# aliabdelkader/FusionTransformer

Hardware: AMD Instinct MI355X
Metric: frames/sec fwd+bwd (SemanticKITTI synth), whole job (higher is better)
Workload: dtype f32

## Files before the change

fusiontransformer_amd/_lib.py:

```python
from __future__ import annotations

import ctypes as C
import os

import torch

_HERE = os.path.dirname(os.path.abspath(__file__))
LIB_PATH = os.path.join(_HERE, "csrc", "libftx.so")

_i32, _i64, _f32, _vp, _sz = C.c_int32, C.c_int64, C.c_float, C.c_void_p, C.c_size_t

SIGNATURES = {
    "ftx_version": (C.c_int, []),
    "ftx_last_error": (C.c_char_p, []),
    "ftx_stream_scratch_bytes": (_sz, []),
    "ftx_stream_scratch_attach": (C.c_int, [_vp, _vp, _sz]),
    "ftx_stream_scratch_reset": (C.c_int, [_vp]),
    "ftx_stream_scratch_release": (C.c_int, [_vp]),
    "ftx_hash": (C.c_int, [_vp, _i64, _vp, _vp]),
    "ftx_hash_kernel": (C.c_int, [_vp, _i64, _vp, _i32, _vp, _vp]),
    "ftx_floor_coords": (C.c_int, [_vp, _i64, _i32, _vp, _vp]),
    "ftx_hashtable_capacity": (_i64, [_i64]),
    "ftx_hashtable_build": (C.c_int, [_vp, _i64, _vp, _vp, _i64, _vp]),
    "ftx_hashtable_query": (C.c_int, [_vp, _i64, _vp, _vp, _i64, _vp, _vp]),
# ... 75 lines not shown
    "ftx_bn_train_fwd": (C.c_int, [_vp, _vp, _vp, _vp, _vp, _vp, _f32, _f32, _i64, _i32, _i32, _vp, _vp, _vp, _vp, _sz, _vp]),
    "ftx_bn_eval_fwd": (C.c_int, [_vp, _vp, _vp, _vp, _vp, _vp, _f32, _i64, _i32, _i32, _vp, _vp]),
    "ftx_adam_chunk_elements": (_i32, []),
    "ftx_adam_tensor_bytes": (_i32, []),
    "ftx_adam_step": (C.c_int, [_vp, _vp, _vp, _i32, C.c_double, C.c_double, _f32, _f32, _vp]),
    "ftx_add_layernorm_fwd": (C.c_int, [_vp, _vp, _vp, _vp, _vp, _f32, _i64, _i32, _vp, _vp, _vp, _vp, _vp]),
    "ftx_layernorm_bwd_workspace_bytes": (_sz, [_i64, _i32]),
    "ftx_add_layernorm_bwd": (C.c_int, [_vp, _vp, _vp, _vp, _vp, _vp, _i64, _i32, _i32, _vp, _vp, _vp, _sz, _vp]),
    "ftx_colsum_workspace_bytes": (_sz, [_i64, _i32]),
    "ftx_colsum": (C.c_int, [_vp, _i64, _i32, _vp, _vp, _sz, _vp]),
    "ftx_attn_fwd": (C.c_int, [_vp, _i32, _i32, _i32, _i32, _f32, _vp, _vp, _vp]),
    "ftx_attn_bwd_workspace_bytes": (_sz, [_i32, _i32, _i32]),
    "ftx_attn_bwd": (C.c_int, [_vp, _vp, _vp, _vp, _i32, _i32, _i32, _i32, _f32, _vp, _vp, _sz, _vp]),
    "ftx_attn_fwd_tiled": (C.c_int, [_vp, _i32, _i32, _i32, _i32, _f32, _vp, _vp, _i32, _i32, _vp]),
    "ftx_attn_bwd_tiled": (C.c_int, [_vp, _vp, _vp, _vp, _i32, _i32, _i32, _i32, _f32, _vp, _vp, _sz, _i32, _i32, _vp]),
    "ftx_attn_fwd_bf16": (C.c_int, [_vp, _i32, _i32, _i32, _i32, _f32, _vp, _vp, _i32, _i32, _vp]),
    "ftx_attn_bwd_bf16": (C.c_int, [_vp, _vp, _vp, _vp, _i32, _i32, _i32, _i32, _f32, _vp, _vp, _sz, _i32, _i32, _vp]),
    "ftx_attn_split_tiling_built": (_i32, [_i32, _i32, _i32]),
    "ftx_attn_fwd_split": (C.c_int, [_vp, _i32, _i32, _i32, _i32, _f32, _vp, _vp, _i32, _i32, _vp]),
    "ftx_attn_bwd_split": (C.c_int, [_vp, _vp, _vp, _vp, _i32, _i32, _i32, _i32, _f32, _vp, _vp, _sz, _i32, _i32, _vp]),
    "ftx_dense_gemm_bf16": (C.c_int, [_vp, _vp, _i32, _vp, _vp, _i64, _i32, _i32, _i32, _vp, _vp, _vp]),
    "ftx_dense_wgrad_bf16_workspace_bytes": (_sz, [_i64, _i32, _i32]),
    "ftx_dense_wgrad_bf16": (C.c_int, [_vp, _vp, _i64, _i32, _i32, _vp, _vp, _sz, _vp]),
    "ftx_dense_bf16_tile": (C.c_int, [_i32, _i64, _i32, _i32, _vp, _vp, _vp]),
    "ftx_dense_gemm_split": (C.c_int, [_vp, _vp, _i32, _vp, _vp, _i64, _i32, _i32, _i32, _vp, _vp, _vp]),
    "ftx_dense_wgrad_split_workspace_bytes": (_sz, [_i64, _i32, _i32]),
    "ftx_dense_wgrad_split": (C.c_int, [_vp, _vp, _i64, _i32, _i32, _vp, _vp, _sz, _vp]),
    "ftx_dense_split_tile": (C.c_int, [_i32, _i64, _i32, _i32, _vp, _vp, _vp]),
    "ftx_fusion_loss_workspace_bytes": (_sz, []),
    "ftx_fusion_loss": (C.c_int, [_vp, _vp, _vp, _vp, _vp, _vp, _f32, _i64, _i32, _i32, _vp, _vp, _vp, _vp, _vp, _vp, _vp, _vp, _sz, _vp]),
# ... 99 lines not shown
```

fusiontransformer_amd/csrc/ftx_attn.hip:

```cpp
#include "ftx_common.h"
#include "ftx_mfma.h"
#include "ftx_split.h"

using namespace ftx;

constexpr int HD = 64;
constexpr int TS = 68;
constexpr float LOG2E = 1.4426950408889634f;
constexpr float LN2 = 0.6931471805599453f;

__device__ inline int acc_row(int g, int h) { return (g & 3) + 8 * (g >> 2) + 4 * h; }

__device__ inline float exp2_raw(float x) { return __builtin_amdgcn_exp2f(x); }

__device__ inline const float *qkv_row(const float *qkv, int b, int t, int which, int hd, int T, int nh) {
  return qkv + ((((int64_t)b * T + t) * 3 + which) * nh + hd) * HD;
}

struct AttnF32 {
  using Frag = float[32];
  template <int NT> using Stage = float4[512 / NT];
  using X = f32x16;
  static constexpr int tile_floats(bool row, bool col) { return 32 * TS; }

// ... 339 lines not shown
#pragma unroll
      for (int t = 0; t < NTILES; ++t)
#pragma unroll
        for (int g = 0; g < 16; ++g) cw[(t * 16 + g) * 64] = acc[t][g];
    }
    __syncthreads();
    if ((grp & (2 * s - 1)) == 0 && grp + s < SPLIT) {
#pragma unroll
      for (int t = 0; t < NTILES; ++t)
#pragma unroll
        for (int g = 0; g < 16; ++g) acc[t][g] += cw[(t * 16 + g) * 64];
    }
  }
}

template <class P, int QW, int SPLIT>
__device__ inline void attn_fwd_body(const float *__restrict__ qkv, int T, int nh, float scale, float *__restrict__ out, float *__restrict__ lse) {
  constexpr int NT = 64 * QW, KF = P::tile_floats(true, false), GROUP = KF + P::tile_floats(false, true);
  __shared__ __attribute__((aligned(16))) float smem[smem_floats<QW, SPLIT, 34, GROUP>()];
  const int tid = threadIdx.x % NT, grp = threadIdx.x / NT;
  float *Ks = smem + grp * GROUP, *Vs = Ks + KF;
  const int wave = tid >> 6, lane = tid & 63, l31 = lane & 31, h = lane >> 5;
  const int hd = blockIdx.y, b = blockIdx.z;
  const int q = blockIdx.x * (32 * QW) + wave * 32 + l31;
  const bool qv = q < T;
  const bool wave_live = blockIdx.x * (32 * QW) + wave * 32 < T;
  const float sl2 = scale * LOG2E;

  typename P::Frag qf;
  P::load_frag(qkv_row(qkv, b, qv ? q : 0, 0, hd, T, nh), h, qv, qf);
  P::fold(qf, sl2);

// ... 16 lines not shown
      P::template prefetch<NT>(qkv, b, hd, 1, (kt + SPLIT) * 32, T, nh, tid, rk);
      P::template prefetch<NT>(qkv, b, hd, 2, (kt + SPLIT) * 32, T, nh, tid, rv);
    }
    if (kt < ntiles && wave_live) {
      f32x16 st;
#pragma unroll
      for (int g = 0; g < 16; ++g) st[g] = 0.f;
      P::first(Ks, l31, h, qf, st);
#pragma unroll
      for (int g = 0; g < 16; ++g) st[g] = P::score(st[g], sl2);
      if (kt == ntiles - 1) {
#pragma unroll
        for (int g = 0; g < 16; ++g)
          if (kt * 32 + acc_row(g, h) >= T) st[g] = -INFINITY;
      }
      float mx = fmaxf(fmaxf(fmaxf(st[0], st[1]), fmaxf(st[2], st[3])), fmaxf(fmaxf(st[4], st[5]), fmaxf(st[6], st[7])));
      mx = fmaxf(mx, fmaxf(fmaxf(fmaxf(st[8], st[9]), fmaxf(st[10], st[11])), fmaxf(fmaxf(st[12], st[13]), fmaxf(st[14], st[15]))));
      mx = fmaxf(mx, __shfl_xor(mx, 32, 64));
      const float m_new = fmaxf(m, mx);
      float rs = 0.f;
#pragma unroll
      for (int g = 0; g < 16; ++g) {
        float p = exp2_raw(st[g] - m_new);
        st[g] = p;
        rs += p;
      }
      rs += __shfl_xor(rs, 32, 64);
      if (__any(m_new != m)) {
        const float alpha = exp2_raw(m - m_new);
        l *= alpha;
// ... 219 lines not shown
    group_sync<QW>();
  }
  merge_sum<QW, SPLIT, 2>(smem, grp, wave, lane, acc);
  if (qv && grp == 0) {
    float *qp = gqkv + ((((int64_t)b * T + q) * 3 + 0) * nh + hd) * HD;
#pragma unroll
    for (int g4 = 0; g4 < 4; ++g4) {
      int r = acc_row(4 * g4, h);
      *(float4 *)(qp + r) = make_float4(acc[0][4 * g4], acc[0][4 * g4 + 1], acc[0][4 * g4 + 2], acc[0][4 * g4 + 3]);
      *(float4 *)(qp + 32 + r) = make_float4(acc[1][4 * g4], acc[1][4 * g4 + 1], acc[1][4 * g4 + 2], acc[1][4 * g4 + 3]);
    }
  }
}

template <int QW, int SPLIT>
__global__ __launch_bounds__(64 * QW * SPLIT) void attn_fwd_kernel(const float *__restrict__ qkv, int T, int nh, float scale, float *__restrict__ out,
    float *__restrict__ lse) {
  attn_fwd_body<AttnF32, QW, SPLIT>(qkv, T, nh, scale, out, lse);
}
template <int QW, int SPLIT>
__global__ __launch_bounds__(64 * QW * SPLIT) void attn_bwd_kv_kernel(const float *__restrict__ qkv, const float *__restrict__ go,
    const float *__restrict__ lse, const float *__restrict__ delta, int T, int nh, float scale, float *__restrict__ gqkv) {
  attn_bwd_kv_body<AttnF32, QW, SPLIT>(qkv, go, lse, delta, T, nh, scale, gqkv);
}
template <int QW, int SPLIT>
__global__ __launch_bounds__(64 * QW * SPLIT) void attn_bwd_q_kernel(const float *__restrict__ qkv, const float *__restrict__ go,
    const float *__restrict__ lse, const float *__restrict__ delta, int T, int nh, float scale, float *__restrict__ gqkv) {
  attn_bwd_q_body<AttnF32, QW, SPLIT>(qkv, go, lse, delta, T, nh, scale, gqkv);
}
__global__ void attn_delta_kernel(const float *__restrict__ o, const float *__restrict__ go, int64_t rows, int T, int nh, float *__restrict__ delta) {
  attn_delta_body<AttnF32>(o, go, rows, T, nh, delta);
}
template <int QW, int SPLIT>
__global__ __launch_bounds__(64 * QW * SPLIT) void attn_fwd_bf16_kernel(const float *__restrict__ qkv, int T, int nh, float scale, float *__restrict__ out,
    float *__restrict__ lse) {
  attn_fwd_body<AttnBf16, QW, SPLIT>(qkv, T, nh, scale, out, lse);
}
template <int QW, int SPLIT>
__global__ __launch_bounds__(64 * QW * SPLIT) void attn_bwd_kv_bf16_kernel(const float *__restrict__ qkv, const float *__restrict__ go,
    const float *__restrict__ lse, const float *__restrict__ delta, int T, int nh, float scale, float *__restrict__ gqkv) {
  attn_bwd_kv_body<AttnBf16, QW, SPLIT>(qkv, go, lse, delta, T, nh, scale, gqkv);
}
template <int QW, int SPLIT>
__global__ __launch_bounds__(64 * QW * SPLIT) void attn_bwd_q_bf16_kernel(const float *__restrict__ qkv, const float *__restrict__ go,
    const float *__restrict__ lse, const float *__restrict__ delta, int T, int nh, float scale, float *__restrict__ gqkv) {
  attn_bwd_q_body<AttnBf16, QW, SPLIT>(qkv, go, lse, delta, T, nh, scale, gqkv);
// ... 159 lines not shown
}
extern "C" int ftx_attn_bwd_bf16(const float *qkv, const float *out, const float *grad_out, const float *lse, int32_t b, int32_t t, int32_t h,
                                 int32_t d, float scale, float *grad_qkv, void *workspace, size_t workspace_bytes, int32_t qw, int32_t split,
                                 void *stream) {
  return attn_bwd_entry<AttnBf16Family>(qkv, out, grad_out, lse, b, t, h, d, scale, grad_qkv, workspace, workspace_bytes, qw, split, stream);
}
extern "C" int ftx_attn_fwd_split(const float *qkv, int32_t b, int32_t t, int32_t h, int32_t d, float scale, float *out, float *lse, int32_t qw,
                                  int32_t split, void *stream) {
  return attn_fwd_entry<AttnSplitFamily>(qkv, b, t, h, d, scale, out, lse, qw, split, stream);
}
extern "C" int ftx_attn_bwd_split(const float *qkv, const float *out, const float *grad_out, const float *lse, int32_t b, int32_t t, int32_t h,
                                  int32_t d, float scale, float *grad_qkv, void *workspace, size_t workspace_bytes, int32_t qw, int32_t split,
                                  void *stream) {
  return attn_bwd_entry<AttnSplitFamily>(qkv, out, grad_out, lse, b, t, h, d, scale, grad_qkv, workspace, workspace_bytes, qw, split, stream);
}
```

fusiontransformer_amd/csrc/ftx_exec_vit_train.hip:

```cpp
#include <algorithm>
#include <mutex>
#include <string>
#include <unordered_map>
#include "ftx_vit_tables.h"

using namespace ftx;
using namespace ftx::vit;

namespace {

struct Saved {
  int64_t s, stats1, h, qkv, att, lse, s2, stats2, h2, pre, act;
};
struct Plan {
  int64_t rows = 0, tokens = 0;
  Saved blk[kMaxBlocks];
  int64_t g[3] = {0, 0, 0}, dpre = 0, gqkv = 0, ws = 0, stage = 0, total = 0;
  size_t ws_attn = 0, ws_ln = 0, ws_col_d = 0, ws_col_h = 0, ws_col_q = 0;
  size_t ws_w2[2] = {0, 0}, ws_w1[2] = {0, 0}, ws_wp[2] = {0, 0}, ws_wq[2] = {0, 0};
};

void make_plan(const Model &M, int32_t b, int32_t n_seg, Plan &P) {
  P.tokens = tokens_of(M);
  P.rows = (int64_t)b * P.tokens;
  const int64_t rows = P.rows;
  const int32_t D = M.dim, H = M.hidden;
  const int64_t row = align256(4 * rows * D), wide = align256(4 * rows * H);
  const int64_t stats = align256(8 * rows), lse = align256(4 * (int64_t)b * M.heads * P.tokens);
  Offsets256 off;
  for (int k = 0; k < n_seg; ++k) {
    Saved &S = P.blk[k];
    S.s = k ? off.take(row) : -1;
    S.stats1 = off.take(stats);
    S.h = off.take(row);
    S.qkv = off.take(3 * row);
    S.att = off.take(row);
    S.lse = off.take(lse);
    S.s2 = off.take(row);
    S.stats2 = off.take(stats);
    S.h2 = off.take(row);
    S.pre = off.take(wide);
    S.act = off.take(wide);
  }
  for (int j = 0; j < 3; ++j) P.g[j] = off.take(row);
  P.dpre = off.take(wide);
  P.gqkv = off.take(3 * row);
  P.ws_attn = ftx_attn_bwd_workspace_bytes(b, (int32_t)P.tokens, M.heads);
  P.ws_ln = ftx_layernorm_bwd_workspace_bytes(rows, D);
  P.ws_col_d = ftx_colsum_workspace_bytes(rows, D);
  P.ws_col_h = ftx_colsum_workspace_bytes(rows, H);
  P.ws_col_q = ftx_colsum_workspace_bytes(rows, 3 * D);
  P.ws_w2[0] = ftx_dense_wgrad_split_workspace_bytes(rows, D, H);
  P.ws_w2[1] = ftx_dense_wgrad_bf16_workspace_bytes(rows, D, H);
  P.ws_w1[0] = ftx_dense_wgrad_split_workspace_bytes(rows, H, D);
  P.ws_w1[1] = ftx_dense_wgrad_bf16_workspace_bytes(rows, H, D);
  P.ws_wp[0] = ftx_dense_wgrad_split_workspace_bytes(rows, D, D);
  P.ws_wp[1] = ftx_dense_wgrad_bf16_workspace_bytes(rows, D, D);
  P.ws_wq[0] = ftx_dense_wgrad_split_workspace_bytes(rows, 3 * D, D);
  P.ws_wq[1] = ftx_dense_wgrad_bf16_workspace_bytes(rows, 3 * D, D);
  size_t ws = std::max({P.ws_attn, P.ws_ln, P.ws_col_d, P.ws_col_h, P.ws_col_q});
  for (int j = 0; j < 2; ++j) ws = std::max({ws, P.ws_w2[j], P.ws_w1[j], P.ws_wp[j], P.ws_wq[j]});
  P.ws = off.take((int64_t)ws);
  P.stage = off.take(4 * 3 * (int64_t)D);
  P.total = off.end < 256 ? 256 : off.end;
}

struct Note {
  int32_t b, first, last, linear_mode, attn_mode, dim, tokens;
  bool backward_ran;
};
std::mutex g_mu;
std::unordered_map<const void *, Note> g_note;

int fail(const char *who, const char *what, int block, int rc) {
  const std::string inner = ftx_last_error();
// ... 76 lines not shown
  auto attn = attn_mode == 2 ? ftx_attn_fwd_split : attn_mode == 1 ? ftx_attn_fwd_bf16 : ftx_attn_fwd_tiled;
  float *m = at(P.g[0]), *proj = at(P.g[1]);
  const float *r = x_in;
  for (int i = block_first; i <= block_last; ++i) {
    const Block &B = blocks[i];
    const Saved &S = P.blk[i - block_first];
    float *mean1 = at(S.stats1), *mean2 = at(S.stats2);
    const float *s = r;
    if (i == block_first) {
      RUN("norm1", ftx_add_layernorm_fwd(r, nullptr, nullptr, B.norm1_w, B.norm1_b, M.eps, rows, dim, nullptr, at(S.h), mean1, mean1 + rows, stream));
    } else {
      RUN("norm1", ftx_add_layernorm_fwd(r, m, blocks[i - 1].fc2_b, B.norm1_w, B.norm1_b, M.eps, rows, dim, at(S.s), at(S.h), mean1, mean1 + rows, stream));
      s = at(S.s);
    }
    RUN("qkv", gemm(at(S.h), B.qkv_w, 0, B.qkv_b, nullptr, rows, 3 * dim, dim, FTX_EPI_BIAS, at(S.qkv), nullptr, stream));
    RUN("attention", attn(at(S.qkv), b, T, M.heads, 64, 0.125f, at(S.att), at(S.lse), 0, 0, stream));
    RUN("proj", gemm(at(S.att), B.proj_w, 0, nullptr, nullptr, rows, dim, dim, FTX_EPI_NONE, proj, nullptr, stream));
    RUN("norm2", ftx_add_layernorm_fwd(s, proj, B.proj_b, B.norm2_w, B.norm2_b, M.eps, rows, dim, at(S.s2), at(S.h2), mean2, mean2 + rows, stream));
    RUN("fc1", gemm(at(S.h2), B.fc1_w, 0, B.fc1_b, nullptr, rows, M.hidden, dim, FTX_EPI_BIAS_GELU, at(S.act), at(S.pre), stream));
    RUN("fc2", gemm(at(S.act), B.fc2_w, 0, nullptr, nullptr, rows, dim, M.hidden, FTX_EPI_NONE, m, nullptr, stream));
    r = at(S.s2);
  }
  {
    const int i = block_last;
    RUN("materialise", ftx_rows_add_bias(r, m, blocks[i].fc2_b, rows, dim, x_out, stream));
  }
  {
    std::lock_guard<std::mutex> lock(g_mu);
    g_note[arena] = Note{b, block_first, block_last, linear_mode, attn_mode, dim, (int32_t)P.tokens, false};
  }
  return FTX_OK;
// ... 59 lines not shown
    RUN("fc1 data gradient", gemm(dpre, B.fc1_w, 1, nullptr, nullptr, rows, dim, hid, FTX_EPI_NONE, gb, nullptr, stream));
    RUN("fc1 weight gradient", wgrad(dpre, at(S.h2), rows, hid, dim, (float *)G.fc1_w, ws, P.ws_w1[lm], stream));
    RUN("fc1 bias gradient", ftx_colsum(dpre, rows, hid, (float *)G.fc1_b, ws, P.ws_col_h, stream));
    {
      const bool direct = together(G.norm2_w, G.norm2_b, G.proj_b);
      float *gp = direct ? (float *)G.norm2_w : stage;
      RUN("norm2 backward", ftx_add_layernorm_bwd(gb, gs, at(S.s2), B.norm2_w, mean2, mean2 + rows, rows, dim, 1, gc, gp, ws, P.ws_ln, stream));
      if (!direct) {
        RUN("norm2 weight gradient", ftx_rows_add_bias(stage, nullptr, nullptr, 1, dim, (float *)G.norm2_w, stream));
        RUN("norm2 bias gradient", ftx_rows_add_bias(stage + dim, nullptr, nullptr, 1, dim, (float *)G.norm2_b, stream));
        RUN("proj bias gradient", ftx_rows_add_bias(stage + 2 * dim, nullptr, nullptr, 1, dim, (float *)G.proj_b, stream));
      }
    }
    RUN("proj data gradient", gemm(gc, B.proj_w, 1, nullptr, nullptr, rows, dim, dim, FTX_EPI_NONE, ga, nullptr, stream));
    RUN("proj weight gradient", wgrad(gc, at(S.att), rows, dim, dim, (float *)G.proj_w, ws, P.ws_wp[lm], stream));
    RUN("attention backward", attn(at(S.qkv), at(S.att), ga, at(S.lse), b, T, M.heads, 64, 0.125f, gqkv, ws, P.ws_attn, 0, 0, stream));
    RUN("qkv data gradient", gemm(gqkv, B.qkv_w, 1, nullptr, nullptr, rows, dim, 3 * dim, FTX_EPI_NONE, gb, nullptr, stream));
    RUN("qkv weight gradient", wgrad(gqkv, at(S.h), rows, 3 * dim, dim, (float *)G.qkv_w, ws, P.ws_wq[lm], stream));
    RUN("qkv bias gradient", ftx_colsum(gqkv, rows, 3 * dim, (float *)G.qkv_b, ws, P.ws_col_q, stream));
    {
      float *gprev = first ? nullptr : (float *)grads[i - 1].fc2_b;
      const bool direct = together(G.norm1_w, G.norm1_b, gprev);
      float *gp = direct ? (float *)G.norm1_w : stage;
      RUN("norm1 backward", ftx_add_layernorm_bwd(gb, first ? nullptr : gc, s, B.norm1_w, mean1, mean1 + rows, rows, dim, first ? 0 : 1, ga, gp, ws, P.ws_ln, stream));
      if (!direct) {
        RUN("norm1 weight gradient", ftx_rows_add_bias(stage, nullptr, nullptr, 1, dim, (float *)G.norm1_w, stream));
        RUN("norm1 bias gradient", ftx_rows_add_bias(stage + dim, nullptr, nullptr, 1, dim, (float *)G.norm1_b, stream));
        if (gprev) RUN("fc2 bias gradient", ftx_rows_add_bias(stage + 2 * dim, nullptr, nullptr, 1, dim, gprev, stream));
      }
    }
    if (first) RUN("input gradient", ftx_rows_add(gc, ga, rows, dim, grad_in, stream));
// ... 6 lines not shown
```

fusiontransformer_amd/functional.py:

```python
from __future__ import annotations

import ctypes
import functools

import numpy as np
import torch

from . import _lib
from ._lib import check, ptr, req, stream

I32, I64, F32 = torch.int32, torch.int64, torch.float32


def _empty(shape, dtype, like):
    return torch.empty(shape, dtype=dtype, device=like.device)


_SCRATCH = {}
_WS_BYTES = {}


def _ws_bytes(fn_name, *args):
    key = (fn_name,) + args
    v = _WS_BYTES.get(key)
# ... 1328 lines not shown
    rows, cols = x.shape
    out = _empty((cols,), F32, x)
    ws_bytes = _ws_bytes("ftx_colsum_workspace_bytes", rows, cols)
    ws = _scratch(ws_bytes, x)
    check(L.ftx_colsum(ptr(x), rows, cols, ptr(out), ptr(ws), ws_bytes, stream()), "ftx_colsum")
    return out


_ATTENTION = {FP32: ("ftx_attn_fwd_tiled", "attn_fwd", "ftx_attn_bwd_tiled", "attn_bwd"),
              BF16: ("ftx_attn_fwd_bf16", "attn_fwd_bf16", "ftx_attn_bwd_bf16", "attn_bwd_bf16"),
              SPLIT: ("ftx_attn_fwd_split", "attn_fwd_split", "ftx_attn_bwd_split", "attn_bwd_split")}


class _Attention(torch.autograd.Function):
    @staticmethod
    def forward(ctx, qkv, scale, tiling=(0, 0), bf16=False):
        L = _lib.load()
        fn, kind = _ATTENTION[bf16][:2]
        qkv = req(qkv.contiguous(), F32, "attention qkv", 5)
        b, t, three, h, d = qkv.shape
        if three != 3 or d != 64:
            raise ValueError(f"attention: qkv must be (B, T, 3, heads, 64), got {tuple(qkv.shape)}")
        out = _empty((b, t, h * d), F32, qkv)
        lse = _empty((b, h, t), F32, qkv)
        qw, split = int(tiling[0]), int(tiling[1])
        _log_launch(kind, dict(b=b, t=t, h=h, d=d, products=2), lambda: check(getattr(L, fn)(
            ptr(qkv), b, t, h, d, float(scale), ptr(out), ptr(lse), qw, split, stream()), fn))
        ctx.save_for_backward(qkv, out, lse)
        ctx.scale, ctx.tiling, ctx.bf16 = float(scale), (qw, split), bf16
        return out

    @staticmethod
    def backward(ctx, go):
        L = _lib.load()
        fn, kind = _ATTENTION[ctx.bf16][2:]
        qkv, out, lse = ctx.saved_tensors
        b, t, _, h, d = qkv.shape
        go = req(go.contiguous(), F32, "attention grad", 3)
        gqkv = torch.empty_like(qkv)
        ws_bytes = int(L.ftx_attn_bwd_workspace_bytes(b, t, h))
        ws = torch.empty((ws_bytes,), dtype=torch.uint8, device=qkv.device)
        _log_launch(kind, dict(b=b, t=t, h=h, d=d, products=7), lambda: check(getattr(L, fn)(
            ptr(qkv), ptr(out), ptr(go), ptr(lse), b, t, h, d, ctx.scale, ptr(gqkv), ptr(ws), ws_bytes, ctx.tiling[0], ctx.tiling[1], stream()), fn))
        return gqkv, None, None, None


def attention(qkv, scale, tiling=(0, 0), bf16=False, operands=None):
    return _Attention.apply(qkv, scale, tiling, operand_mode(bf16, operands))


EPI_NONE, EPI_BIAS, EPI_BIAS_GELU, EPI_DGELU = 0, 1, 2, 3
_DENSE_MODES = ("bf16", "split")


def vit_linear_supported(x, weight):
    n, k = weight.shape
    return (x.is_cuda and weight.is_cuda and x.dtype == F32 and weight.dtype == F32 and x.shape[-1] == k and k % 64 == 0 and n % 64 == 0
            and x.numel() // k <= (1 << 30))


def _dense_gemm(a, w, w_kn, epi, bias=None, pre_in=None, with_pre=False, mode="bf16"):
    L = _lib.load()
    m, kr = a.shape
# ... 404 lines not shown
```

fusiontransformer_amd/models/transformers.py:

```python
from __future__ import annotations

import contextlib
import gc
from functools import partial
from typing import Dict

import torch
import torch.nn as nn
import torch.nn.functional as F

__all__ = ["Image2DTransformer", "image_2d_distilled_transformer", "SpatialTransformer", "ScaleUpModule"]


_ONES = {}


def _ones_row(m, like):
    key = (m, like.device, like.dtype)
    if key not in _ONES:
        _ONES[key] = torch.ones(1, m, device=like.device, dtype=like.dtype)
    return _ONES[key]


class _LinearFn(torch.autograd.Function):
# ... 116 lines not shown
        super().__init__()
        self.num_heads = num_heads
        head_dim = dim // num_heads
        self.scale = head_dim ** -0.5
        self.qkv = nn.Linear(dim, dim * 3, bias=qkv_bias)
        self.attn_drop = nn.Dropout(attn_drop)
        self.proj = nn.Linear(dim, dim)
        self.proj_drop = nn.Dropout(proj_drop)
        self.attn_impl = "ftx"

    def forward(self, x, with_proj_bias=True):
        B, N, C = x.shape
        qkv = _linear(x, self.qkv)
        if self.attn_impl in ATTN_OPERANDS:
            from .. import functional as spf
            x = spf.attention(qkv.view(B, N, 3, self.num_heads, C // self.num_heads), self.scale, operands=ATTN_OPERANDS[self.attn_impl])
        else:
            qkv = qkv.reshape(B, N, 3, self.num_heads, C // self.num_heads).permute(2, 0, 3, 1, 4)
            q, k, v = qkv[0], qkv[1], qkv[2]
            attn = (q @ k.transpose(-2, -1)) * self.scale
            attn = attn.softmax(dim=-1)
            attn = self.attn_drop(attn)
            x = (attn @ v).transpose(1, 2).reshape(B, N, C)
        return self.proj_drop(_linear(x, self.proj, with_proj_bias))


class Block(nn.Module):
    def __init__(self, dim, num_heads, mlp_ratio=4.0, qkv_bias=True, norm_layer=nn.LayerNorm):
        super().__init__()
        self.norm1 = norm_layer(dim)
        self.attn = Attention(dim, num_heads=num_heads, qkv_bias=qkv_bias)
# ... 495 lines not shown
```

include/ftx.h:

```cpp
#ifndef FTX_H
#define FTX_H

#include <stddef.h>
#include <stdint.h>

#ifdef __cplusplus
extern "C" {
#endif

#define FTX_OK 0
#define FTX_EINVAL -1
#define FTX_ELAUNCH -2
#define FTX_EWORKSPACE -3

int ftx_version(void);
const char *ftx_last_error(void);

size_t ftx_stream_scratch_bytes(void);
int ftx_stream_scratch_attach(void *stream, void *buffer, size_t bytes);
int ftx_stream_scratch_reset(void *stream);
int ftx_stream_scratch_release(void *stream);


int ftx_hash(const int32_t *coords, int64_t n, int64_t *out, void *stream);
// ... 124 lines not shown
int ftx_adam_step(const void *table, const int32_t *chunk_tensor, const int64_t *chunk_offset, int32_t n_chunks, double beta1, double beta2, float eps, float weight_decay, void *stream);

int ftx_add_layernorm_fwd(const float *x, const float *y, const float *y_bias, const float *gamma, const float *beta, float eps, int64_t rows, int32_t c, float *s_out, float *h_out, float *mean, float *rstd, void *stream);
size_t ftx_layernorm_bwd_workspace_bytes(int64_t rows, int32_t c);
int ftx_add_layernorm_bwd(const float *grad_h, const float *grad_s, const float *s, const float *gamma, const float *mean, const float *rstd, int64_t rows, int32_t c, int32_t with_y_bias, float *grad_x, float *grad_params, void *workspace, size_t workspace_bytes, void *stream);

size_t ftx_colsum_workspace_bytes(int64_t rows, int32_t cols);
int ftx_colsum(const float *x, int64_t rows, int32_t cols, float *out, void *workspace, size_t workspace_bytes, void *stream);


int ftx_attn_fwd(const float *qkv, int32_t b, int32_t t, int32_t h, int32_t d, float scale, float *out, float *lse, void *stream);
size_t ftx_attn_bwd_workspace_bytes(int32_t b, int32_t t, int32_t h);
int ftx_attn_bwd(const float *qkv, const float *out, const float *grad_out, const float *lse, int32_t b, int32_t t, int32_t h, int32_t d, float scale, float *grad_qkv, void *workspace, size_t workspace_bytes, void *stream);
int ftx_attn_fwd_tiled(const float *qkv, int32_t b, int32_t t, int32_t h, int32_t d, float scale, float *out, float *lse, int32_t qw, int32_t split, void *stream);
int ftx_attn_bwd_tiled(const float *qkv, const float *out, const float *grad_out, const float *lse, int32_t b, int32_t t, int32_t h, int32_t d, float scale, float *grad_qkv, void *workspace, size_t workspace_bytes, int32_t qw, int32_t split, void *stream);
int ftx_attn_fwd_bf16(const float *qkv, int32_t b, int32_t t, int32_t h, int32_t d, float scale, float *out, float *lse, int32_t qw, int32_t split, void *stream);
int ftx_attn_bwd_bf16(const float *qkv, const float *out, const float *grad_out, const float *lse, int32_t b, int32_t t, int32_t h, int32_t d, float scale, float *grad_qkv, void *workspace, size_t workspace_bytes, int32_t qw, int32_t split, void *stream);
int32_t ftx_attn_split_tiling_built(int32_t qw, int32_t split, int32_t backward);
int ftx_attn_fwd_split(const float *qkv, int32_t b, int32_t t, int32_t h, int32_t d, float scale, float *out, float *lse, int32_t qw, int32_t split, void *stream);
int ftx_attn_bwd_split(const float *qkv, const float *out, const float *grad_out, const float *lse, int32_t b, int32_t t, int32_t h, int32_t d, float scale, float *grad_qkv, void *workspace, size_t workspace_bytes, int32_t qw, int32_t split, void *stream);

#define FTX_EPI_NONE 0
#define FTX_EPI_BIAS 1
#define FTX_EPI_BIAS_GELU 2
#define FTX_EPI_DGELU 3
int ftx_dense_gemm_bf16(const float *A, const float *W, int32_t w_kn, const float *bias, const float *pre_in, int64_t m, int32_t n, int32_t k, int32_t epilogue, float *out, float *pre_out, void *stream);
size_t ftx_dense_wgrad_bf16_workspace_bytes(int64_t m, int32_t n, int32_t k);
int ftx_dense_wgrad_bf16(const float *dY, const float *X, int64_t m, int32_t n, int32_t k, float *dW, void *workspace, size_t workspace_bytes, void *stream);
int ftx_dense_bf16_tile(int32_t form, int64_t m, int32_t n, int32_t k, int32_t *tile_m_host, int32_t *tile_n_host, int32_t *split_host);

// ... 95 lines not shown
```

Before: 150.6.

## Store attention score tiles in forward and reuse them in backward

The forward attention kernel gains a variant that writes the scaled pre-softmax score tiles to global memory. A new backward path reads these tiles instead of recomputing QK^T. It computes dS once in the KV kernel, stores it, and has the Q kernel read dS back rather than recompute scores. This trades the QK^T recompute in backward for O(T^2) extra memory traffic and storage per block and head, and it is enabled by default for fp32 training.

```diff
diff --git a/fusiontransformer_amd/_lib.py b/fusiontransformer_amd/_lib.py
--- a/fusiontransformer_amd/_lib.py
+++ b/fusiontransformer_amd/_lib.py
@@ -113,6 +113,10 @@
     "ftx_attn_bwd": (C.c_int, [_vp, _vp, _vp, _vp, _i32, _i32, _i32, _i32, _f32, _vp, _vp, _sz, _vp]),
     "ftx_attn_fwd_tiled": (C.c_int, [_vp, _i32, _i32, _i32, _i32, _f32, _vp, _vp, _i32, _i32, _vp]),
     "ftx_attn_bwd_tiled": (C.c_int, [_vp, _vp, _vp, _vp, _i32, _i32, _i32, _i32, _f32, _vp, _vp, _sz, _i32, _i32, _vp]),
+    "ftx_attn_keep_bytes": (_sz, [_i32, _i32, _i32]),
+    "ftx_attn_fwd_keep": (C.c_int, [_vp, _i32, _i32, _i32, _i32, _f32, _vp, _vp, _vp, _i32, _i32, _vp]),
+    "ftx_attn_bwd_kept_workspace_bytes": (_sz, [_i32, _i32, _i32]),
+    "ftx_attn_bwd_kept": (C.c_int, [_vp, _vp, _vp, _vp, _vp, _i32, _i32, _i32, _i32, _f32, _vp, _vp, _sz, _i32, _i32, _vp]),
     "ftx_attn_fwd_bf16": (C.c_int, [_vp, _i32, _i32, _i32, _i32, _f32, _vp, _vp, _i32, _i32, _vp]),
     "ftx_attn_bwd_bf16": (C.c_int, [_vp, _vp, _vp, _vp, _i32, _i32, _i32, _i32, _f32, _vp, _vp, _sz, _i32, _i32, _vp]),
     "ftx_attn_split_tiling_built": (_i32, [_i32, _i32, _i32]),
diff --git a/fusiontransformer_amd/csrc/ftx_attn.hip b/fusiontransformer_amd/csrc/ftx_attn.hip
--- a/fusiontransformer_amd/csrc/ftx_attn.hip
+++ b/fusiontransformer_amd/csrc/ftx_attn.hip
@@ -377,8 +377,42 @@
   }
 }
 
-template <class P, int QW, int SPLIT>
-__device__ inline void attn_fwd_body(const float *__restrict__ qkv, int T, int nh, float scale, float *__restrict__ out, float *__restrict__ lse) {
+constexpr int XS = 36;
+constexpr int XP = 16 * XS;
+struct KeptTile { float4 r0, r1, r2, r3; };
+
+__device__ inline int64_t kept_tile(int b, int hd, int nh, int nt, int qt, int kt) {
+  return ((((int64_t)b * nh + hd) * nt + qt) * nt + kt) * 1024;
+}
+__device__ inline void kept_store(float *tile, int lane, const f32x16 &x) {
+  const int c = lane & 31, h = lane >> 5;
+#pragma unroll
+  for (int j = 0; j < 4; ++j) *(float4 *)(tile + ((j * 32 + c) * 2 + h) * 4) = make_float4(x[4 * j], x[4 * j + 1], x[4 * j + 2], x[4 * j + 3]);
+}
+__device__ inline KeptTile kept_prefetch(const float *tile, int lane) {
+  const float4 *p = (const float4 *)tile + lane;
+  return KeptTile{p[0], p[64], p[128], p[192]};
+}
+__device__ inline f32x16 kept_transpose(float *xp, int lane, const KeptTile r) {
+  const int l31 = lane & 31, h = lane >> 5;
+  f32x16 x;
+#pragma unroll
+  for (int half = 0; half < 2; ++half) {
+    group_sync<1>();
+    if (h == half) {
+      float4 *d = (float4 *)(xp + ((lane >> 1) & 15) * XS + 4 * (lane & 1));
+      d[0] = r.r0; d[2] = r.r1; d[4] = r.r2; d[6] = r.r3;
+    }
+    group_sync<1>();
+#pragma unroll
+    for (int g = 0; g < 8; ++g) x[8 * half + g] = xp[(acc_row(8 * half + g, h) - 16 * half) * XS + l31];
+  }
+  return x;
+}
+
+template <class P, int QW, int SPLIT, bool KEEP = false>
+__device__ inline void attn_fwd_body(const float *__restrict__ qkv, int T, int nh, float scale, float *__restrict__ out, float *__restrict__ lse,
+                                     float *__restrict__ keep = nullptr) {
   constexpr int NT = 64 * QW, KF = P::tile_floats(true, false), GROUP = KF + P::tile_floats(false, true);
   __shared__ __attribute__((aligned(16))) float smem[smem_floats<QW, SPLIT, 34, GROUP>()];
   const int tid = threadIdx.x % NT, grp = threadIdx.x / NT;
@@ -425,6 +459,7 @@
         for (int g = 0; g < 16; ++g)
           if (kt * 32 + acc_row(g, h) >= T) st[g] = -INFINITY;
       }
+      if constexpr (KEEP) kept_store(keep + kept_tile(b, hd, nh, ntiles, blockIdx.x * QW + wave, kt), lane, st);
       float mx = fmaxf(fmaxf(fmaxf(st[0], st[1]), fmaxf(st[2], st[3])), fmaxf(fmaxf(st[4], st[5]), fmaxf(st[6], st[7])));
       mx = fmaxf(mx, fmaxf(fmaxf(fmaxf(st[8], st[9]), fmaxf(st[10], st[11])), fmaxf(fmaxf(st[12], st[13]), fmaxf(st[14], st[15]))));
       mx = fmaxf(mx, __shfl_xor(mx, 32, 64));
@@ -674,6 +709,154 @@
 }
 
 template <int QW, int SPLIT>
+__device__ inline void attn_bwd_kv_kept_body(const float *__restrict__ qkv, const float *__restrict__ go, const float *__restrict__ lse,
+                                             const float *__restrict__ delta, const float *__restrict__ s_keep, int T, int nh, float scale,
+                                             float *__restrict__ gqkv, float *__restrict__ ds) {
+  using P = AttnF32;
+  constexpr int NT = 64 * QW, TF = P::tile_floats(true, true), GROUP = 2 * TF + 64, TILES = smem_floats<QW, SPLIT, 64, GROUP>();
+  __shared__ __attribute__((aligned(16))) float smem[TILES + QW * SPLIT * XP];
+  const int tid = threadIdx.x % NT, grp = threadIdx.x / NT;
+  float *Qs = smem + grp * GROUP, *Gs = Qs + TF, *s_lse = Gs + TF, *s_delta = s_lse + 32, *xp = smem + TILES + (threadIdx.x >> 6) * XP;
+  const int wave = tid >> 6, lane = tid & 63, l31 = lane & 31, h = lane >> 5;
+  const int hd = blockIdx.y, b = blockIdx.z;
+  const int ktile = blockIdx.x * QW + wave;
+  const int key = ktile * 32 + l31;
+  const bool kv = key < T;
+  const bool wave_live = ktile * 32 < T;
+
+  typename P::Frag vf;
+  P::load_frag(qkv_row(qkv, b, kv ? key : 0, 2, hd, T, nh), h, kv, vf);
+
+  f32x16 acc[4];
+#pragma unroll
+  for (int t = 0; t < 4; ++t)
+#pragma unroll
+    for (int g = 0; g < 16; ++g) acc[t][g] = 0.f;
+
+  const int ntiles = (T + 31) / 32;
+  const int iters = (ntiles + SPLIT - 1) / SPLIT;
+  typename P::template Stage<NT> rq, rg;
+  KeptTile rs = {};
+  P::template prefetch<NT>(qkv, b, hd, 0, grp * 32, T, nh, tid, rq);
+  P::template prefetch_o<NT>(go, b, hd, grp * 32, T, nh, tid, rg);
+  if (wave_live && grp < ntiles) rs = kept_prefetch(s_keep + kept_tile(b, hd, nh, ntiles, grp, ktile), lane);
+  for (int it = 0; it < iters; ++it) {
+    const int qt = it * SPLIT + grp;
+    const bool live = qt < ntiles && wave_live;
+    P::template store<NT, false, true>(Qs, tid, rq);
+    P::template store<NT, true, true>(Gs, tid, rg);
+    if (tid < 32) {
+      int t = qt * 32 + tid;
+      s_lse[tid] = t < T ? lse[((int64_t)b * nh + hd) * T + t] * LOG2E : 0.f;
+      s_delta[tid] = t < T ? delta[((int64_t)b * nh + hd) * T + t] : 0.f;
+    }
+    group_sync<QW>();
+    f32x16 s = {};
+    if (live) s = kept_transpose(xp, lane, rs);
+    if (it + 1 < iters) {
+      P::template prefetch<NT>(qkv, b, hd, 0, (qt + SPLIT) * 32, T, nh, tid, rq);
+      P::template prefetch_o<NT>(go, b, hd, (qt + SPLIT) * 32, T, nh, tid, rg);
+      if (wave_live && qt + SPLIT < ntiles) rs = kept_prefetch(s_keep + kept_tile(b, hd, nh, ntiles, qt + SPLIT, ktile), lane);
+    }
+    if (live) {
+      f32x16 dp;
+#pragma unroll
+      for (int g = 0; g < 16; ++g) dp[g] = 0.f;
+      P::first(Gs, l31, h, vf, dp);
+#pragma unroll
+      for (int g = 0; g < 16; ++g) {
+        const int r = acc_row(g, h);
+        const float p = exp2_raw(s[g] - s_lse[r]);
+        s[g] = p;
+        dp[g] = p * (dp[g] - s_delta[r]) * scale;
+      }
+      if (qt == ntiles - 1) {
+#pragma unroll
+        for (int g = 0; g < 16; ++g)
+          if (qt * 32 + acc_row(g, h) >= T) s[g] = dp[g] = 0.f;
+      }
+      kept_store(ds + kept_tile(b, hd, nh, ntiles, qt, ktile), lane, dp);
+      P::template second<true>(Gs, 0, l31, h, s, acc[0]);
+      P::template second<true>(Gs, 32, l31, h, s, acc[1]);
+      P::template second<false>(Qs, 0, l31, h, dp, acc[2]);
+      P::template second<false>(Qs, 32, l31, h, dp, acc[3]);
+    }
+    group_sync<QW>();
+  }
+  merge_sum<QW, SPLIT, 4>(smem, grp, wave, lane, acc);
+  if (kv && grp == 0) {
+    float *kp = gqkv + ((((int64_t)b * T + key) * 3 + 1) * nh + hd) * HD;
+    float *vp = gqkv + ((((int64_t)b * T + key) * 3 + 2) * nh + hd) * HD;
+#pragma unroll
+    for (int g4 = 0; g4 < 4; ++g4) {
+      int r = acc_row(4 * g4, h);
+      *(float4 *)(vp + r) = make_float4(acc[0][4 * g4], acc[0][4 * g4 + 1], acc[0][4 * g4 + 2], acc[0][4 * g4 + 3]);
+      *(float4 *)(vp + 32 + r) = make_float4(acc[1][4 * g4], acc[1][4 * g4 + 1], acc[1][4 * g4 + 2], acc[1][4 * g4 + 3]);
+      *(float4 *)(kp + r) = make_float4(acc[2][4 * g4], acc[2][4 * g4 + 1], acc[2][4 * g4 + 2], acc[2][4 * g4 + 3]);
+      *(float4 *)(kp + 32 + r) = make_float4(acc[3][4 * g4], acc[3][4 * g4 + 1], acc[3][4 * g4 + 2], acc[3][4 * g4 + 3]);
+    }
+  }
+}
+
+template <int QW, int SPLIT>
+__device__ inline void attn_bwd_q_kept_body(const float *__restrict__ qkv, const float *__restrict__ ds, int T, int nh, float *__restrict__ gqkv) {
+  using P = AttnF32;
+  constexpr int NT = 64 * QW, GROUP = P::tile_floats(false, true), TILES = smem_floats<QW, SPLIT, 32, GROUP>();
+  __shared__ __attribute__((aligned(16))) float smem[TILES + QW * SPLIT * XP];
+  const int tid = threadIdx.x % NT, grp = threadIdx.x / NT;
+  float *Ks = smem + grp * GROUP, *xp = smem + TILES + (threadIdx.x >> 6) * XP;
+  const int wave = tid >> 6, lane = tid & 63, l31 = lane & 31, h = lane >> 5;
+  const int hd = blockIdx.y, b = blockIdx.z;
+  const int qtile = blockIdx.x * QW + wave;
+  const int q = qtile * 32 + l31;
+  const bool qv = q < T;
+  const bool wave_live = qtile * 32 < T;
+
+  f32x16 acc[2];
+#pragma unroll
+  for (int g = 0; g < 16; ++g) acc[0][g] = acc[1][g] = 0.f;
+
+  const int ntiles = (T + 31) / 32;
+  const int iters = (ntiles + SPLIT - 1) / SPLIT;
+  typename P::template Stage<NT> rk;
+  KeptTile rd = {};
+  P::template prefetch<NT>(qkv, b, hd, 1, grp * 32, T, nh, tid, rk);
+  if (wave_live && grp < ntiles) rd = kept_prefetch(ds + kept_tile(b, hd, nh, ntiles, qtile, grp), lane);
+  for (int it = 0; it < iters; ++it) {
+    const int kt = it * SPLIT + grp;
+    const bool live = kt < ntiles && wave_live;
+    P::template store<NT, false, true>(Ks, tid, rk);
+    group_sync<QW>();
+    f32x16 dst = {};
+    if (live) dst = kept_transpose(xp, lane, rd);
+    if (it + 1 < iters) {
+      P::template prefetch<NT>(qkv, b, hd, 1, (kt + SPLIT) * 32, T, nh, tid, rk);
+      if (wave_live && kt + SPLIT < ntiles) rd = kept_prefetch(ds + kept_tile(b, hd, nh, ntiles, qtile, kt + SPLIT), lane);
+    }
+    if (live) {
+      if (kt == ntiles - 1) {
+#pragma unroll
+        for (int g = 0; g < 16; ++g)
+          if (kt * 32 + acc_row(g, h) >= T) dst[g] = 0.f;
+      }
+      P::template second<false>(Ks, 0, l31, h, dst, acc[0]);
+      P::template second<false>(Ks, 32, l31, h, dst, acc[1]);
+    }
+    group_sync<QW>();
+  }
+  merge_sum<QW, SPLIT, 2>(smem, grp, wave, lane, acc);
+  if (qv && grp == 0) {
+    float *qp = gqkv + ((((int64_t)b * T + q) * 3 + 0) * nh + hd) * HD;
+#pragma unroll
+    for (int g4 = 0; g4 < 4; ++g4) {
+      int r = acc_row(4 * g4, h);
+      *(float4 *)(qp + r) = make_float4(acc[0][4 * g4], acc[0][4 * g4 + 1], acc[0][4 * g4 + 2], acc[0][4 * g4 + 3]);
+      *(float4 *)(qp + 32 + r) = make_float4(acc[1][4 * g4], acc[1][4 * g4 + 1], acc[1][4 * g4 + 2], acc[1][4 * g4 + 3]);
+    }
+  }
+}
+
+template <int QW, int SPLIT>
 __global__ __launch_bounds__(64 * QW * SPLIT) void attn_fwd_kernel(const float *__restrict__ qkv, int T, int nh, float scale, float *__restrict__ out,
     float *__restrict__ lse) {
   attn_fwd_body<AttnF32, QW, SPLIT>(qkv, T, nh, scale, out, lse);
@@ -690,6 +873,22 @@
 }
 __global__ void attn_delta_kernel(const float *__restrict__ o, const float *__restrict__ go, int64_t rows, int T, int nh, float *__restrict__ delta) {
   attn_delta_body<AttnF32>(o, go, rows, T, nh, delta);
+}
+template <int QW, int SPLIT>
+__global__ __launch_bounds__(64 * QW * SPLIT) void attn_fwd_keep_kernel(const float *__restrict__ qkv, int T, int nh, float scale, float *__restrict__ out,
+    float *__restrict__ lse, float *__restrict__ s_keep) {
+  attn_fwd_body<AttnF32, QW, SPLIT, true>(qkv, T, nh, scale, out, lse, s_keep);
+}
+template <int QW, int SPLIT>
+__global__ __launch_bounds__(64 * QW * SPLIT) void attn_bwd_kv_kept_kernel(const float *__restrict__ qkv, const float *__restrict__ go,
+    const float *__restrict__ lse, const float *__restrict__ delta, const float *__restrict__ s_keep, int T, int nh, float scale,
+    float *__restrict__ gqkv, float *__restrict__ ds) {
+  attn_bwd_kv_kept_body<QW, SPLIT>(qkv, go, lse, delta, s_keep, T, nh, scale, gqkv, ds);
+}
+template <int QW, int SPLIT>
+__global__ __launch_bounds__(64 * QW * SPLIT) void attn_bwd_q_kept_kernel(const float *__restrict__ qkv, const float *__restrict__ ds, int T, int nh,
+    float *__restrict__ gqkv) {
+  attn_bwd_q_kept_body<QW, SPLIT>(qkv, ds, T, nh, gqkv);
 }
 template <int QW, int SPLIT>
 __global__ __launch_bounds__(64 * QW * SPLIT) void attn_fwd_bf16_kernel(const float *__restrict__ qkv, int T, int nh, float scale, float *__restrict__ out,
@@ -879,3 +1078,52 @@
                                   void *stream) {
   return attn_bwd_entry<AttnSplitFamily>(qkv, out, grad_out, lse, b, t, h, d, scale, grad_qkv, workspace, workspace_bytes, qw, split, stream);
 }
+
+static size_t attn_kept_tiles_bytes(int32_t b, int32_t t, int32_t h) {
+  const size_t nt = (size_t)ceil_div(t, 32);
+  return sizeof(float) * 1024 * nt * nt * (size_t)b * (size_t)h;
+}
+extern "C" size_t ftx_attn_keep_bytes(int32_t b, int32_t t, int32_t h) {
+  if (b <= 0 || t <= 0 || h <= 0) return 256;
+  return attn_kept_tiles_bytes(b, t, h);
+}
+static size_t attn_kept_delta_bytes(int32_t b, int32_t t, int32_t h) { return (sizeof(float) * (size_t)b * t * h + 255) / 256 * 256; }
+extern "C" size_t ftx_attn_bwd_kept_workspace_bytes(int32_t b, int32_t t, int32_t h) {
+  if (b <= 0 || t <= 0 || h <= 0) return 256;
+  return attn_kept_delta_bytes(b, t, h) + attn_kept_tiles_bytes(b, t, h);
+}
+
+extern "C" int ftx_attn_fwd_keep(const float *qkv, int32_t b, int32_t t, int32_t h, int32_t d, float scale, float *out, float *lse, float *s_keep,
+                                 int32_t qw, int32_t split, void *stream) {
+  const char *me = "ftx_attn_fwd_keep";
+  int rc = attn_check(me, b, t, h, d);
+  if (rc != FTX_OK) return rc;
+  FTX_REQUIRE(qkv && out && lse && s_keep, "%s: null pointer", me);
+  FTX_REQUIRE(((uintptr_t)s_keep & 15) == 0, "%s: s_keep must be 16-byte aligned", me);
+  FTX_REQUIRE(AttnF32Family::built(qw, split, false), "%s: (%d, %d) is not a built tiling", me, qw, split);
+  hipStream_t st = (hipStream_t)stream;
+  AttnF32Family::config(b, t, h, false, qw, split);
+  ATTN_DISPATCH(attn_fwd_keep_kernel, qkv, t, h, scale, out, lse, s_keep);
+  return check_launch(me);
+}
+
+extern "C" int ftx_attn_bwd_kept(const float *qkv, const float *out, const float *grad_out, const float *lse, const float *s_keep, int32_t b, int32_t t,
+                                 int32_t h, int32_t d, float scale, float *grad_qkv, void *workspace, size_t workspace_bytes, int32_t qw, int32_t split,
+                                 void *stream) {
+  const char *me = "ftx_attn_bwd_kept";
+  int rc = attn_check(me, b, t, h, d);
+  if (rc != FTX_OK) return rc;
+  FTX_REQUIRE(qkv && out && grad_out && lse && s_keep && grad_qkv && workspace, "%s: null pointer", me);
+  FTX_REQUIRE(((uintptr_t)s_keep & 15) == 0 && ((uintptr_t)workspace & 15) == 0, "%s: s_keep and workspace must be 16-byte aligned", me);
+  FTX_REQUIRE(AttnF32Family::built(qw, split, true), "%s: (%d, %d) is not a built tiling", me, qw, split);
+  if (workspace_bytes < ftx_attn_bwd_kept_workspace_bytes(b, t, h)) return workspace_short(me, workspace_bytes, ftx_attn_bwd_kept_workspace_bytes(b, t, h));
+  hipStream_t st = (hipStream_t)stream;
+  float *delta = (float *)workspace;
+  float *ds = (float *)((char *)workspace + attn_kept_delta_bytes(b, t, h));
+  const int64_t rows = (int64_t)b * t * h;
+  attn_delta_kernel<<<(unsigned)ceil_div(rows * 16, 256), 256, 0, st>>>(out, grad_out, rows, t, h, delta);
+  AttnF32Family::config(b, t, h, true, qw, split);
+  ATTN_DISPATCH(attn_bwd_kv_kept_kernel, qkv, grad_out, lse, delta, s_keep, t, h, scale, grad_qkv, ds);
+  ATTN_DISPATCH(attn_bwd_q_kept_kernel, qkv, ds, t, h, grad_qkv);
+  return check_launch(me);
+}
diff --git a/fusiontransformer_amd/csrc/ftx_exec_vit_train.hip b/fusiontransformer_amd/csrc/ftx_exec_vit_train.hip
--- a/fusiontransformer_amd/csrc/ftx_exec_vit_train.hip
+++ b/fusiontransformer_amd/csrc/ftx_exec_vit_train.hip
@@ -10,13 +10,13 @@
 namespace {
 
 struct Saved {
-  int64_t s, stats1, h, qkv, att, lse, s2, stats2, h2, pre, act;
+  int64_t s, stats1, h, qkv, att, lse, keep, s2, stats2, h2, pre, act;
 };
 struct Plan {
   int64_t rows = 0, tokens = 0;
   Saved blk[kMaxBlocks];
   int64_t g[3] = {0, 0, 0}, dpre = 0, gqkv = 0, ws = 0, stage = 0, total = 0;
-  size_t ws_attn = 0, ws_ln = 0, ws_col_d = 0, ws_col_h = 0, ws_col_q = 0;
+  size_t ws_attn = 0, ws_attn_kept = 0, ws_ln = 0, ws_col_d = 0, ws_col_h = 0, ws_col_q = 0;
   size_t ws_w2[2] = {0, 0}, ws_w1[2] = {0, 0}, ws_wp[2] = {0, 0}, ws_wq[2] = {0, 0};
 };
 
@@ -27,6 +27,7 @@
   const int32_t D = M.dim, H = M.hidden;
   const int64_t row = align256(4 * rows * D), wide = align256(4 * rows * H);
   const int64_t stats = align256(8 * rows), lse = align256(4 * (int64_t)b * M.heads * P.tokens);
+  const int64_t keep = align256((int64_t)ftx_attn_keep_bytes(b, (int32_t)P.tokens, M.heads));
   Offsets256 off;
   for (int k = 0; k < n_seg; ++k) {
     Saved &S = P.blk[k];
@@ -36,6 +37,7 @@
     S.qkv = off.take(3 * row);
     S.att = off.take(row);
     S.lse = off.take(lse);
+    S.keep = off.take(keep);
     S.s2 = off.take(row);
     S.stats2 = off.take(stats);
     S.h2 = off.take(row);
@@ -46,6 +48,7 @@
   P.dpre = off.take(wide);
   P.gqkv = off.take(3 * row);
   P.ws_attn = ftx_attn_bwd_workspace_bytes(b, (int32_t)P.tokens, M.heads);
+  P.ws_attn_kept = ftx_attn_bwd_kept_workspace_bytes(b, (int32_t)P.tokens, M.heads);
   P.ws_ln = ftx_layernorm_bwd_workspace_bytes(rows, D);
   P.ws_col_d = ftx_colsum_workspace_bytes(rows, D);
   P.ws_col_h = ftx_colsum_workspace_bytes(rows, H);
@@ -58,7 +61,7 @@
   P.ws_wp[1] = ftx_dense_wgrad_bf16_workspace_bytes(rows, D, D);
   P.ws_wq[0] = ftx_dense_wgrad_split_workspace_bytes(rows, 3 * D, D);
   P.ws_wq[1] = ftx_dense_wgrad_bf16_workspace_bytes(rows, 3 * D, D);
-  size_t ws = std::max({P.ws_attn, P.ws_ln, P.ws_col_d, P.ws_col_h, P.ws_col_q});
+  size_t ws = std::max({P.ws_attn, P.ws_attn_kept, P.ws_ln, P.ws_col_d, P.ws_col_h, P.ws_col_q});
   for (int j = 0; j < 2; ++j) ws = std::max({ws, P.ws_w2[j], P.ws_w1[j], P.ws_wp[j], P.ws_wq[j]});
   P.ws = off.take((int64_t)ws);
   P.stage = off.take(4 * 3 * (int64_t)D);
@@ -165,7 +168,11 @@
       s = at(S.s);
     }
     RUN("qkv", gemm(at(S.h), B.qkv_w, 0, B.qkv_b, nullptr, rows, 3 * dim, dim, FTX_EPI_BIAS, at(S.qkv), nullptr, stream));
-    RUN("attention", attn(at(S.qkv), b, T, M.heads, 64, 0.125f, at(S.att), at(S.lse), 0, 0, stream));
+    if (attn_mode == 0) {
+      RUN("attention", ftx_attn_fwd_keep(at(S.qkv), b, T, M.heads, 64, 0.125f, at(S.att), at(S.lse), at(S.keep), 0, 0, stream));
+    } else {
+      RUN("attention", attn(at(S.qkv), b, T, M.heads, 64, 0.125f, at(S.att), at(S.lse), 0, 0, stream));
+    }
     RUN("proj", gemm(at(S.att), B.proj_w, 0, nullptr, nullptr, rows, dim, dim, FTX_EPI_NONE, proj, nullptr, stream));
     RUN("norm2", ftx_add_layernorm_fwd(s, proj, B.proj_b, B.norm2_w, B.norm2_b, M.eps, rows, dim, at(S.s2), at(S.h2), mean2, mean2 + rows, stream));
     RUN("fc1", gemm(at(S.h2), B.fc1_w, 0, B.fc1_b, nullptr, rows, M.hidden, dim, FTX_EPI_BIAS_GELU, at(S.act), at(S.pre), stream));
@@ -255,7 +262,11 @@
     }
     RUN("proj data gradient", gemm(gc, B.proj_w, 1, nullptr, nullptr, rows, dim, dim, FTX_EPI_NONE, ga, nullptr, stream));
     RUN("proj weight gradient", wgrad(gc, at(S.att), rows, dim, dim, (float *)G.proj_w, ws, P.ws_wp[lm], stream));
-    RUN("attention backward", attn(at(S.qkv), at(S.att), ga, at(S.lse), b, T, M.heads, 64, 0.125f, gqkv, ws, P.ws_attn, 0, 0, stream));
+    if (attn_mode == 0) {
+      RUN("attention backward", ftx_attn_bwd_kept(at(S.qkv), at(S.att), ga, at(S.lse), at(S.keep), b, T, M.heads, 64, 0.125f, gqkv, ws, P.ws_attn_kept, 0, 0, stream));
+    } else {
+      RUN("attention backward", attn(at(S.qkv), at(S.att), ga, at(S.lse), b, T, M.heads, 64, 0.125f, gqkv, ws, P.ws_attn, 0, 0, stream));
+    }
     RUN("qkv data gradient", gemm(gqkv, B.qkv_w, 1, nullptr, nullptr, rows, dim, 3 * dim, FTX_EPI_NONE, gb, nullptr, stream));
     RUN("qkv weight gradient", wgrad(gqkv, at(S.h), rows, 3 * dim, dim, (float *)G.qkv_w, ws, P.ws_wq[lm], stream));
     RUN("qkv bias gradient", ftx_colsum(gqkv, rows, 3 * dim, (float *)G.qkv_b, ws, P.ws_col_q, stream));
diff --git a/fusiontransformer_amd/functional.py b/fusiontransformer_amd/functional.py
--- a/fusiontransformer_amd/functional.py
+++ b/fusiontransformer_amd/functional.py
@@ -1366,9 +1366,10 @@
 
 class _Attention(torch.autograd.Function):
     @staticmethod
-    def forward(ctx, qkv, scale, tiling=(0, 0), bf16=False):
+    def forward(ctx, qkv, scale, tiling=(0, 0), bf16=False, keep=False):
         L = _lib.load()
         fn, kind = _ATTENTION[bf16][:2]
+        keep = bool(keep) and bf16 == FP32
         qkv = req(qkv.contiguous(), F32, "attention qkv", 5)
         b, t, three, h, d = qkv.shape
         if three != 3 or d != 64:
@@ -1376,29 +1377,43 @@
         out = _empty((b, t, h * d), F32, qkv)
         lse = _empty((b, h, t), F32, qkv)
         qw, split = int(tiling[0]), int(tiling[1])
-        _log_launch(kind, dict(b=b, t=t, h=h, d=d, products=2), lambda: check(getattr(L, fn)(
-            ptr(qkv), b, t, h, d, float(scale), ptr(out), ptr(lse), qw, split, stream()), fn))
-        ctx.save_for_backward(qkv, out, lse)
-        ctx.scale, ctx.tiling, ctx.bf16 = float(scale), (qw, split), bf16
+        if keep:
+            s_keep = torch.empty((int(L.ftx_attn_keep_bytes(b, t, h)),), dtype=torch.uint8, device=qkv.device)
+            _log_launch("attn_fwd_keep", dict(b=b, t=t, h=h, d=d, products=2), lambda: check(L.ftx_attn_fwd_keep(
+                ptr(qkv), b, t, h, d, float(scale), ptr(out), ptr(lse), ptr(s_keep), qw, split, stream()), "ftx_attn_fwd_keep"))
+            ctx.save_for_backward(qkv, out, lse, s_keep)
+        else:
+            _log_launch(kind, dict(b=b, t=t, h=h, d=d, products=2), lambda: check(getattr(L, fn)(
+                ptr(qkv), b, t, h, d, float(scale), ptr(out), ptr(lse), qw, split, stream()), fn))
+            ctx.save_for_backward(qkv, out, lse)
+        ctx.scale, ctx.tiling, ctx.bf16, ctx.keep = float(scale), (qw, split), bf16, keep
         return out
 
     @staticmethod
     def backward(ctx, go):
         L = _lib.load()
         fn, kind = _ATTENTION[ctx.bf16][2:]
-        qkv, out, lse = ctx.saved_tensors
+        qkv, out, lse = ctx.saved_tensors[:3]
         b, t, _, h, d = qkv.shape
         go = req(go.contiguous(), F32, "attention grad", 3)
         gqkv = torch.empty_like(qkv)
+        if ctx.keep:
+            s_keep = ctx.saved_tensors[3]
+            ws_bytes = int(L.ftx_attn_bwd_kept_workspace_bytes(b, t, h))
+            ws = torch.empty((ws_bytes,), dtype=torch.uint8, device=qkv.device)
+            _log_launch("attn_bwd_kept", dict(b=b, t=t, h=h, d=d, products=4), lambda: check(L.ftx_attn_bwd_kept(
+                ptr(qkv), ptr(out), ptr(go), ptr(lse), ptr(s_keep), b, t, h, d, ctx.scale, ptr(gqkv), ptr(ws), ws_bytes, ctx.tiling[0], ctx.tiling[1],
+                stream()), "ftx_attn_bwd_kept"))
+            return gqkv, None, None, None, None
         ws_bytes = int(L.ftx_attn_bwd_workspace_bytes(b, t, h))
         ws = torch.empty((ws_bytes,), dtype=torch.uint8, device=qkv.device)
         _log_launch(kind, dict(b=b, t=t, h=h, d=d, products=7), lambda: check(getattr(L, fn)(
             ptr(qkv), ptr(out), ptr(go), ptr(lse), b, t, h, d, ctx.scale, ptr(gqkv), ptr(ws), ws_bytes, ctx.tiling[0], ctx.tiling[1], stream()), fn))
-        return gqkv, None, None, None
-
-
-def attention(qkv, scale, tiling=(0, 0), bf16=False, operands=None):
-    return _Attention.apply(qkv, scale, tiling, operand_mode(bf16, operands))
+        return gqkv, None, None, None, None
+
+
+def attention(qkv, scale, tiling=(0, 0), bf16=False, operands=None, keep=False):
+    return _Attention.apply(qkv, scale, tiling, operand_mode(bf16, operands), keep)
 
 
 EPI_NONE, EPI_BIAS, EPI_BIAS_GELU, EPI_DGELU = 0, 1, 2, 3
diff --git a/fusiontransformer_amd/models/transformers.py b/fusiontransformer_amd/models/transformers.py
--- a/fusiontransformer_amd/models/transformers.py
+++ b/fusiontransformer_amd/models/transformers.py
@@ -154,7 +154,9 @@
         qkv = _linear(x, self.qkv)
         if self.attn_impl in ATTN_OPERANDS:
             from .. import functional as spf
-            x = spf.attention(qkv.view(B, N, 3, self.num_heads, C // self.num_heads), self.scale, operands=ATTN_OPERANDS[self.attn_impl])
+            keep = self.attn_impl == "ftx" and self.training and torch.is_grad_enabled() and qkv.is_cuda and qkv.dtype == torch.float32
+            x = spf.attention(qkv.view(B, N, 3, self.num_heads, C // self.num_heads), self.scale, operands=ATTN_OPERANDS[self.attn_impl],
+                              **({"keep": True} if keep else {}))
         else:
             qkv = qkv.reshape(B, N, 3, self.num_heads, C // self.num_heads).permute(2, 0, 3, 1, 4)
             q, k, v = qkv[0], qkv[1], qkv[2]
diff --git a/include/ftx.h b/include/ftx.h
--- a/include/ftx.h
+++ b/include/ftx.h
@@ -162,6 +162,10 @@
 int ftx_attn_bwd(const float *qkv, const float *out, const float *grad_out, const float *lse, int32_t b, int32_t t, int32_t h, int32_t d, float scale, float *grad_qkv, void *workspace, size_t workspace_bytes, void *stream);
 int ftx_attn_fwd_tiled(const float *qkv, int32_t b, int32_t t, int32_t h, int32_t d, float scale, float *out, float *lse, int32_t qw, int32_t split, void *stream);
 int ftx_attn_bwd_tiled(const float *qkv, const float *out, const float *grad_out, const float *lse, int32_t b, int32_t t, int32_t h, int32_t d, float scale, float *grad_qkv, void *workspace, size_t workspace_bytes, int32_t qw, int32_t split, void *stream);
+size_t ftx_attn_keep_bytes(int32_t b, int32_t t, int32_t h);
+int ftx_attn_fwd_keep(const float *qkv, int32_t b, int32_t t, int32_t h, int32_t d, float scale, float *out, float *lse, float *s_keep, int32_t qw, int32_t split, void *stream);
+size_t ftx_attn_bwd_kept_workspace_bytes(int32_t b, int32_t t, int32_t h);
+int ftx_attn_bwd_kept(const float *qkv, const float *out, const float *grad_out, const float *lse, const float *s_keep, int32_t b, int32_t t, int32_t h, int32_t d, float scale, float *grad_qkv, void *workspace, size_t workspace_bytes, int32_t qw, int32_t split, void *stream);
 int ftx_attn_fwd_bf16(const float *qkv, int32_t b, int32_t t, int32_t h, int32_t d, float scale, float *out, float *lse, int32_t qw, int32_t split, void *stream);
 int ftx_attn_bwd_bf16(const float *qkv, const float *out, const float *grad_out, const float *lse, int32_t b, int32_t t, int32_t h, int32_t d, float scale, float *grad_qkv, void *workspace, size_t workspace_bytes, int32_t qw, int32_t split, void *stream);
 int32_t ftx_attn_split_tiling_built(int32_t qw, int32_t split, int32_t backward);
```

Result: no change. 153.3, median of 6 (+1.8%).
